# danielSanchezQ/dkg

Hardware: AMD Instinct MI355X
Metric: verified shares/sec (whole node) at n=1024,t=511; full-ceremony wall time (higher is better)
Workload: dtype u32 (GF(2^255-19), Z_l); 1 GPU; one DKG ceremony n=1024, t=511 (share gen + round-2/4 checks + finalise); n=1024, t=511, parallelism=single GPU, verify_streams=2, rounds_2_4_fused=True, degree_split=4, recombination=short lattice multipliers, recombination_addends=affine Niels, stepping_additions=dedicated (complete redo where exceptional)

## Files before the change

dkg_amd/csrc/kernels.hip:

```cpp
#ifdef DKG_FE_ILP
#define dkgk dkgk_ilp
#endif
#include "kernels.h"
#include "split.h"

#include <algorithm>
#include <cmath>
#include <type_traits>
#include "points.h"

namespace dkgk {

constexpr int COMB_WORDS = AFF_WORDS * COMB_ENTRIES;

#ifndef DKG_DECODE_WAVES
#define DKG_DECODE_WAVES 2
#endif
__global__ __launch_bounds__(256, DKG_DECODE_WAVES) void k_decode(const uint32_t* __restrict__ comp, size_t count,
                                                uint32_t* __restrict__ ext, size_t stride,
                                                uint8_t* __restrict__ ok, size_t pm_N, size_t pm_npad,
                                                uint32_t nseg, uint32_t seg, size_t pm_L, size_t pm_pstride) {
  size_t e = (size_t)blockIdx.x * blockDim.x + threadIdx.x;
  if (e >= count) return;
  uint32_t w[8];
// ... 421 lines not shown
  tab += (size_t)blockIdx.y * G::WORDS;
  ge_p3 b, m;
  pt_load(b, ext, stride, e0 + blockIdx.y);
  for (int i = 0; i < BITS * w; i++) ge_dbl<true>(b, b);
  mul_small_uniform(m, b, (uint32_t)d);
  fe zi, x, y, t, d2;
  fe_ld(d2, ge_const::D2);
  fe_invert(zi, m.Z);
  fe_mul(x, m.X, zi);
  fe_mul(y, m.Y, zi);
  uint32_t* out = tab + ((size_t)w * G::ENTRIES + (d - 1)) * COMBW_STRIDE;
  fe_add(t, y, x);
  fe_carry(t, t);
#pragma unroll
  for (int i = 0; i < 10; i++) out[i] = t.v[i];
  fe_sub(t, y, x);
  fe_carry(t, t);
#pragma unroll
  for (int i = 0; i < 10; i++) out[10 + i] = t.v[i];
  fe_mul(t, x, y);
  fe_mul(t, t, d2);
#pragma unroll
  for (int i = 0; i < 10; i++) out[20 + i] = t.v[i];
  out[30] = 0;
  out[31] = 0;
}

static_assert(COMBW_WORDS * 4 == (size_t)(256 / DKG_COMBW_BITS + 1) * (1u << (DKG_COMBW_BITS - 1)) * 32 * 4,
              "runtime.hip COMBW_BYTES must match points.h");
static_assert(CombGeo<COMBW_BITS>::WORDS == COMBW_WORDS, "one comb geometry");

int fixed_base_windows() { return COMBW_WINDOWS; }

template <int BITS>
void build_combw_r(const uint32_t* ext, size_t stride, size_t e0, uint32_t* tab, hipStream_t stream, size_t count) {
  if (!count) return;
  using G = CombGeo<BITS>;
  hipLaunchKernelGGL(k_build_combw<BITS>, dim3((unsigned)G::WINDOWS, (unsigned)count, G::ENTRIES / comb_build_bs<BITS>()),
                     dim3(comb_build_bs<BITS>()), 0, stream, ext, stride, e0, tab);
}

void build_combw(const uint32_t* ext, size_t stride, size_t e0, uint32_t* tab, hipStream_t stream, size_t count) {
  build_combw_r<COMBW_BITS>(ext, stride, e0, tab, stream, count);
}

size_t key_comb_words() { return CombGeo<DKG_KEY_COMB_BITS>::WORDS; }
int key_comb_windows() { return CombGeo<DKG_KEY_COMB_BITS>::WINDOWS; }

void build_key_combs(const uint32_t* ext, size_t stride, size_t e0, uint32_t* tab, hipStream_t stream,
                     size_t count) {
  build_combw_r<DKG_KEY_COMB_BITS>(ext, stride, e0, tab, stream, count);
}

__global__ __launch_bounds__(256) void k_copy_pos(size_t width, size_t npad, size_t N, const uint32_t* __restrict__ C,
                                                  size_t kpos, uint32_t* __restrict__ e, size_t pstride) {
  const size_t dl = (size_t)blockIdx.x * blockDim.x + threadIdx.x;
  if (dl >= width) return;
  const size_t d = blockIdx.y * pstride + dl;
  const size_t S = N * npad;
#pragma unroll 8
  for (int w = 0; w < PT_WORDS; w++) e[w * S + d] = C[w * S + kpos * npad + d];
}

#ifndef DKG_STEP_NT
#define DKG_STEP_NT 0
#endif
#ifndef DKG_AFF_NT
#define DKG_AFF_NT 0
#endif
#ifndef DKG_BINOM_WAVE_NT
#define DKG_BINOM_WAVE_NT 0
#endif
#ifndef DKG_COMB_NT
#define DKG_COMB_NT 0
#endif
template <bool NT>
DKG_DEV void binom_st(uint32_t* p, uint32_t v) {
  if constexpr (NT) __builtin_nontemporal_store(v, p);
  else *p = v;
}
template <bool NT>
DKG_DEV void binom_pt_store(uint32_t* __restrict__ base, size_t stride, size_t e, const ge_p3& p) {
  if constexpr (NT) pt_store_nt(base, stride, e, p);
  else pt_store(base, stride, e, p);
}


#ifndef DKG_BINOM_STEP_WAVES
#define DKG_BINOM_STEP_WAVES 4
#endif
template <bool DED, bool NT, bool IL = false>
__global__ __launch_bounds__(64, IL ? 2 : DKG_BINOM_STEP_WAVES) void k_binom_step(int r, int k, size_t npad, size_t N,
                                                    const uint32_t* __restrict__ C,
                                                    const uint32_t* __restrict__ ein, uint32_t* __restrict__ eout,
                                                    size_t pstride, unsigned gx, unsigned last_piece,
                                                    int last_off, uint32_t* __restrict__ flags, size_t col_base,
                                                    size_t dreal, unsigned gw, int fany) {
  __shared__ uint32_t qs[PT_WORDS * 64];
  uint32_t* q = qs + threadIdx.x;
  const unsigned piece = blockIdx.x / gx, grp = blockIdx.x - piece * gx;
  const size_t d = piece * pstride + (size_t)grp * blockDim.x + threadIdx.x;
  const size_t S = N * npad;
  const int m = r - (int)blockIdx.y;
  if (m == 0) {
#pragma unroll 8
    for (int w = 0; w < PT_WORDS; w++) binom_st<NT>(eout + w * S + d, C[w * S + (size_t)k * npad + d]);
    return;
  }
  const int re = r - (piece == last_piece ? last_off : 0);
  if (m > re) return;
  {
    ge_p3 cur;
    pt_load(cur, ein, S, (size_t)m * npad + d);
    uint32_t keep = (m == re) ? 0u : 0xffffffffu;
    asm volatile("" : "+v"(keep));
    uint32_t* cw = reinterpret_cast<uint32_t*>(&cur);
#pragma unroll
    for (int w = 0; w < PT_WORDS; w++) cw[w] = (cw[w] & keep) | ((w == 10 || w == 20) ? ~keep & 1u : 0u);
    ge_cached cc;
    if constexpr (DED) ge_to_cached_ded(cc, cur);
    else ge_to_cached(cc, cur);
    lds_put_cached(q, cc);
  }
  __builtin_amdgcn_sched_barrier(0);
  ge_p3 x;
  pt_load(x, ein, S, (size_t)(m - 1) * npad + d);
  if constexpr (DED) {
    bool bad = false;
    ge_add_ded_lds(x, x, q);
    bad |= fe_tight_zero(x.Z);
    mul_small_ded_lds<IL || DKG_BINOM_IL != 0>(x, (uint32_t)m, q, bad);
    const size_t gcol = col_base + (size_t)grp * blockDim.x + threadIdx.x;
    const bool real = (gcol / gw) * 64 + (gcol % gw) % 64 < dreal;
    if (__ballot(bad && real) != 0 && threadIdx.x == 0)
      flags[fany ? 0 : (size_t)piece * (pstride / 64) + (col_base / 64) + grp] = 1u;
  } else {
    ge_add_lds<IL>(x, x, q, false);
    mul_small_lds<IL>(x, (uint32_t)m, q);
  }
  binom_pt_store<NT>(eout, S, (size_t)m * npad + d, x);
}

__global__ __launch_bounds__(64, 4) void k_binom_pair(int r, int k, size_t npad, size_t N,
                                                    const uint32_t* __restrict__ C,
                                                    const uint32_t* __restrict__ ein, uint32_t* __restrict__ eout,
                                                    size_t pstride, unsigned gx, unsigned last_piece,
                                                    int last_off) {
  __shared__ uint32_t xb[20 * 64];
  __shared__ uint32_t qs[PT_WORDS * 32];
  const int lane = threadIdx.x;
  const unsigned piece = blockIdx.x / gx, grp = blockIdx.x - piece * gx;
  const size_t d = piece * pstride + (size_t)grp * 32 + (lane >> 1);
  const size_t S = N * npad;
  const int m = r - (int)blockIdx.y;
  if (m == 0) {
    if (lane & 1) return;
#pragma unroll 8
    for (int w = 0; w < PT_WORDS; w++) eout[w * S + d] = C[w * S + (size_t)k * npad + d];
    return;
  }
  const int re = r - (piece == last_piece ? last_off : 0);
  if (m > re) return;
  const pair_ctx c{xb, qs + (lane >> 1), lane & 1, lane};
  {
    ge_p3 cur;
    pt_load(cur, ein, S, (size_t)m * npad + d);
    uint32_t keep = (m == re) ? 0u : 0xffffffffu;
    asm volatile("" : "+v"(keep));
    uint32_t* cw = reinterpret_cast<uint32_t*>(&cur);
#pragma unroll
    for (int w = 0; w < PT_WORDS; w++) cw[w] = (cw[w] & keep) | ((w == 10 || w == 20) ? ~keep & 1u : 0u);
    pair_put_cached(c, cur);
  }
  ge_p3 x;
  pt_load(x, ein, S, (size_t)(m - 1) * npad + d);
  ge_add_pair(x, x, c, false);
  mul_small_pair(x, (uint32_t)m, c);
  if (lane & 1) return;
  pt_store(eout, S, (size_t)m * npad + d, x);
}

void binom_step_pair(size_t r, size_t width, size_t npad, size_t N, const uint32_t* C, const uint32_t* in,
                     uint32_t* out, hipStream_t stream, size_t pieces, size_t pstride, size_t last_len) {
  const int last_off = (last_len && last_len < N) ? (int)(N - last_len) : 0;
  hipLaunchKernelGGL(k_binom_pair, dim3((unsigned)(width / 32 * pieces), (unsigned)(r + 1)), dim3(64), 0, stream,
                     (int)r, (int)(N - 1 - r), npad, N, C, in, out, pstride, (unsigned)(width / 32),
                     (unsigned)(pieces - 1), last_off);
}

void binom_init(size_t width, size_t npad, size_t N, const uint32_t* C, uint32_t* e0, hipStream_t stream,
                size_t pieces, size_t pstride) {
  hipLaunchKernelGGL(k_copy_pos, dim3((unsigned)((width + 255) / 256), (unsigned)pieces), dim3(256), 0, stream, width,
                     npad, N, C, N - 1, e0, pstride);
}

void binom_step(size_t r, size_t width, size_t npad, size_t N, const uint32_t* C, const uint32_t* in, uint32_t* out,
                hipStream_t stream, size_t pieces, size_t pstride, size_t last_len, uint32_t* flags, size_t col_base,
                size_t dreal, unsigned gw, bool flag_any, bool nt, bool il) {
  const int last_off = (last_len && last_len < N) ? (int)(N - last_len) : 0;
  const dim3 grid((unsigned)(width / 64 * pieces), (unsigned)(r + 1));
  auto go = [&](auto kern, uint32_t* fl, int fany) {
    hipLaunchKernelGGL(kern, grid, dim3(64), 0, stream, (int)r, (int)(N - 1 - r), npad, N, C, in, out, pstride,
                       (unsigned)(width / 64), (unsigned)(pieces - 1), last_off, fl, col_base, dreal, gw ? gw : 64u,
                       fany);
  };
  if (il) {
    if (flags && nt) go(k_binom_step<true, true, true>, flags, flag_any ? 1 : 0);
    else if (flags) go(k_binom_step<true, false, true>, flags, flag_any ? 1 : 0);
    else if (nt) go(k_binom_step<false, true, true>, nullptr, 0);
    else go(k_binom_step<false, false, true>, nullptr, 0);
    return;
  }
  if (flags && nt) go(k_binom_step<true, true>, flags, flag_any ? 1 : 0);
  else if (flags) go(k_binom_step<true, false>, flags, flag_any ? 1 : 0);
  else if (nt) go(k_binom_step<false, true>, nullptr, 0);
  else go(k_binom_step<false, false>, nullptr, 0);
}

#ifndef DKG_BINOM_WAVE_CARRY
#define DKG_BINOM_WAVE_CARRY 1
#endif
#ifndef DKG_BINOM_WAVE_WAVES
#define DKG_BINOM_WAVE_WAVES 3
#endif
template <bool CARRY, bool PF, bool DED>
__global__ __launch_bounds__(64, PF ? 2 : (CARRY ? DKG_BINOM_WAVE_WAVES : 4)) void k_binom_wave(int L, size_t npad,
                                                                           const uint32_t* __restrict__ C,
                                                                           uint32_t* e, size_t pstride, unsigned gx,
                                                                           unsigned last_piece, int last_off,
                                                                           uint32_t* eT, uint32_t* __restrict__ flags,
                                                                           size_t col_base, size_t dreal, unsigned gw) {
  static_assert(!PF || CARRY, "the prefetch runs on the carried schedule");
  static_assert(!DED || (CARRY && !PF), "the dedicated pass runs on the carried schedule");
  __shared__ uint32_t qs[PT_WORDS * 64];
  uint32_t* q = qs + threadIdx.x;
  const unsigned piece = blockIdx.x / gx, grp = blockIdx.x - piece * gx;
  const size_t fidx = (size_t)piece * (pstride / 64) + (col_base / 64) + grp;
  if (!DED && flags && !flags[fidx]) return;
  const size_t col0 = piece * pstride + (size_t)grp * 64;
  uint32_t* eb = e + col0;
  const uint32_t* cb = C + col0;
  const uint32_t lane = threadIdx.x;
  const size_t S = (size_t)L * npad;
  const int off = piece == last_piece ? last_off : 0;
  bool bad = false;
  const size_t gcol = col_base + (size_t)grp * 64 + lane;
  const bool real = (gcol / gw) * 64 + (gcol % gw) % 64 < dreal;
  uint32_t* e_top = (L == 1 && eT) ? eT + col0 : eb;
#pragma unroll 8
  for (int w = 0; w < PT_WORDS; w++) e_top[w * S + lane] = cb[w * S + (size_t)(L - 1) * npad + lane];
#pragma unroll 1
  for (int r = 1; r < L; r++) {
    asm volatile("s_waitcnt vmcnt(0)" ::: "memory");
    const int re = r - off;
    ge_p3 carry, nx;
    if constexpr (CARRY) ge_identity(carry);
    if constexpr (PF) {
// ... 41 lines not shown
        if (DKG_BINOM_WAVE_NT) pt_store_nt(eo, S, (size_t)m * npad + lane, x);
        else pt_store(eo, S, (size_t)m * npad + lane, x);
      } else {
        uint32_t* eo = eT + col0 * L;
        asm volatile("" : "+s"(eo));
        pt_store(eo, S, (size_t)lane * L + m, x);
      }
    }
    if (r + 1 < L || !eT) {
#pragma unroll 8
      for (int w = 0; w < PT_WORDS; w++) eb[w * S + lane] = cb[w * S + (size_t)(L - 1 - r) * npad + lane];
    } else {
      uint32_t* eo = eT + col0 * L;
#pragma unroll 8
      for (int w = 0; w < PT_WORDS; w++) eo[w * S + (size_t)lane * L] = cb[w * S + lane];
    }
  }
  if constexpr (DED) {
    if (__ballot(bad && real) != 0 && lane == 0) flags[fidx] = 1u;
  }
}

uint32_t* binomial_wave(size_t width, size_t npad, size_t N, const uint32_t* C, uint32_t* e, hipStream_t stream,
                        size_t pieces, size_t pstride, size_t last_len, uint32_t* eT, bool prefetch,
                        uint32_t* flags, size_t col_base, size_t dreal, unsigned gw) {
  const int last_off = (last_len && last_len < N) ? (int)(N - last_len) : 0;
  const dim3 grid((unsigned)(width / 64 * pieces));
  const unsigned gx = (unsigned)(width / 64), lp = (unsigned)(pieces - 1);
  if (!gw) gw = 64;
  if (prefetch) {
    hipLaunchKernelGGL((k_binom_wave<true, true, false>), grid, dim3(64), 0, stream, (int)N, npad, C, e, pstride, gx,
                       lp, last_off, eT, nullptr, col_base, dreal, gw);
  } else if (flags && DKG_BINOM_WAVE_CARRY) {
    hipLaunchKernelGGL((k_binom_wave<true, false, true>), grid, dim3(64), 0, stream, (int)N, npad, C, e, pstride, gx,
                       lp, last_off, eT, flags, col_base, dreal, gw);
    hipLaunchKernelGGL((k_binom_wave<true, false, false>), grid, dim3(64), 0, stream, (int)N, npad, C, e, pstride,
                       gx, lp, last_off, eT, flags, col_base, dreal, gw);
  } else {
    hipLaunchKernelGGL((k_binom_wave<DKG_BINOM_WAVE_CARRY != 0, false, false>), grid, dim3(64), 0, stream, (int)N,
                       npad, C, e, pstride, gx, lp, last_off, eT, nullptr, col_base, dreal, gw);
  }
  return e;
}

void binomial_wave_redo(size_t width, size_t npad, size_t N, const uint32_t* C, uint32_t* e, hipStream_t stream,
                        size_t pieces, size_t pstride, size_t last_len, uint32_t* flags, size_t col_base,
                        size_t dreal, unsigned gw) {
  const int last_off = (last_len && last_len < N) ? (int)(N - last_len) : 0;
  hipLaunchKernelGGL((k_binom_wave<true, false, false>), dim3((unsigned)(width / 64 * pieces)), dim3(64), 0, stream,
                     (int)N, npad, C, e, pstride, (unsigned)(width / 64), (unsigned)(pieces - 1), last_off, nullptr,
                     flags, col_base, dreal, gw ? gw : 64u);
}

uint32_t* binomial(size_t width, size_t npad, size_t N, const uint32_t* C, uint32_t* e0, uint32_t* e1,
                   hipStream_t stream, size_t pieces, size_t pstride, size_t last_len) {
  binom_init(width, npad, N, C, e0, stream, pieces, pstride);
  uint32_t* in = e0;
  uint32_t* out = e1;
  for (size_t r = 1; r < N; r++) {
    binom_step(r, width, npad, N, C, in, out, stream, pieces, pstride, last_len);
    std::swap(in, out);
  }
  return in;
}


__global__ __launch_bounds__(256) void k_to_column_major(size_t width, size_t npad, size_t N,
                                                         const uint32_t* __restrict__ e, uint32_t* __restrict__ eT,
                                                         size_t pstride) {
  __shared__ uint32_t tile[64][65];
  const size_t w = blockIdx.z % PT_WORDS, base = (blockIdx.z / PT_WORDS) * pstride;
  const size_t c0 = (size_t)blockIdx.x * 64, p0 = (size_t)blockIdx.y * 64;
  const size_t S = N * npad;
  const int tx = threadIdx.x & 63, ty = threadIdx.x >> 6;
#pragma unroll
  for (int i = 0; i < 16; i++) {
    const size_t p = p0 + ty + 4 * i, c = c0 + tx;
    if (p < N && c < width) tile[ty + 4 * i][tx] = e[w * S + p * npad + base + c];
  }
  __syncthreads();
#pragma unroll
  for (int i = 0; i < 16; i++) {
    const size_t c = c0 + ty + 4 * i, p = p0 + tx;
    if (p < N && c < width) eT[w * S + (base + c) * N + p] = tile[tx][ty + 4 * i];
  }
}

void to_column_major(size_t width, size_t npad, size_t N, const uint32_t* e, uint32_t* eT, size_t pieces,
                     size_t pstride, hipStream_t stream) {
  if (!width || !N) return;
  hipLaunchKernelGGL(k_to_column_major,
                     dim3((unsigned)((width + 63) / 64), (unsigned)((N + 63) / 64), (unsigned)(pieces * PT_WORDS)),
                     dim3(256), 0, stream, width, npad, N, e, eT, pstride);
}

__global__ __launch_bounds__(64) void k_zero_tests(size_t count, const uint32_t* __restrict__ limbs,
                                                   uint8_t* __restrict__ out) {
  const size_t e = (size_t)blockIdx.x * 64 + threadIdx.x;
  const bool live = e < count;
  fe a;
#pragma unroll
  for (int i = 0; i < 10; i++) a.v[i] = live ? limbs[10 * e + i] : 1u;
  bool guard = false;
  fe_zero_guard(guard, a, live);
  if (live) {
    out[3 * e] = fe_maybe_zero(a) ? 1 : 0;
    out[3 * e + 1] = fe_tight_zero(a) ? 1 : 0;
    out[3 * e + 2] = guard ? 1 : 0;
  }
}
void zero_tests(size_t count, const uint32_t* limbs, uint8_t* out, hipStream_t stream) {
  if (!count) return;
  hipLaunchKernelGGL(k_zero_tests, dim3((unsigned)((count + 63) / 64)), dim3(64), 0, stream, count, limbs, out);
}

DKG_DEV void fe_ld_raw(fe& r, const uint32_t* __restrict__ p) {
#pragma unroll
  for (int i = 0; i < 10; i++) r.v[i] = p[i];
// ... 1827 lines not shown
```

dkg_amd/csrc/kernels_decl.inc:

```
namespace dkgk {

void decode_points(const uint32_t* comp, size_t count, uint32_t* ext, size_t stride, uint8_t* ok,
                   hipStream_t stream);
void place_position_major(const uint32_t* src, size_t sstride, size_t D, size_t N, size_t npad, uint32_t* out,
                          hipStream_t stream, int nseg = 1, int seg = 0, size_t L = 0, size_t pstride = 0);
void gather_points(const uint32_t* src, size_t sstride, size_t step, size_t k0, size_t count, uint32_t* dst,
                   size_t dstride, hipStream_t stream);
void decode_position_major(const uint32_t* comp, size_t D, size_t N, size_t npad, uint32_t* out, uint8_t* ok,
                           hipStream_t stream, int nseg = 1, int seg = 0, size_t L = 0, size_t pstride = 0);
void fill_identity(size_t S, uint32_t* out, hipStream_t stream);
void check_both(size_t ndealers, size_t nrecv, size_t dealer0, size_t dealer_base, size_t nmod, const uint32_t* s,
                const uint32_t* sp, const uint32_t* R, const uint32_t* tab_g, const uint32_t* tab_h,
                const uint8_t* dok, uint8_t* dec2, uint8_t* dec4, hipStream_t stream, const uint32_t* scale = nullptr,
                size_t j0 = 0, size_t jn = 0, uint32_t* acc = nullptr);
void encode_points(const uint32_t* ext, size_t stride, size_t count, uint32_t* comp, hipStream_t stream);
void build_comb(const uint32_t* ext, size_t stride, size_t e0, uint32_t* tab, hipStream_t stream, size_t count = 1);
void build_combw(const uint32_t* ext, size_t stride, size_t e0, uint32_t* tab, hipStream_t stream, size_t count = 1);

void commit_position_major(size_t D, size_t N, const uint32_t* a, const uint32_t* b, const uint32_t* tab_g,
                           const uint32_t* tab_h, uint32_t* out, size_t W, size_t L, size_t pstride, uint32_t* A0,
                           size_t A0stride, hipStream_t stream);
void commit(size_t count, const uint32_t* a, const uint32_t* b, const uint32_t* tab_g,
            const uint32_t* tab_h, uint32_t* A_ext, uint32_t* E_ext, hipStream_t stream, size_t stride = 0);
void share_eval(size_t D, size_t n, size_t N, const uint32_t* a, const uint32_t* b, uint32_t* s,
                uint32_t* sp, hipStream_t stream);
void poly_eval(size_t D, size_t N, const uint32_t* coeffs, size_t M, const uint32_t* xs, uint32_t* out,
               hipStream_t stream);

uint32_t* binomial(size_t width, size_t npad, size_t N, const uint32_t* C, uint32_t* e0, uint32_t* e1,
                   hipStream_t stream, size_t pieces = 1, size_t pstride = 0, size_t last_len = 0);
void binom_init(size_t width, size_t npad, size_t N, const uint32_t* C, uint32_t* e0, hipStream_t stream,
                size_t pieces = 1, size_t pstride = 0);
void binom_step(size_t r, size_t width, size_t npad, size_t N, const uint32_t* C, const uint32_t* in, uint32_t* out,
                hipStream_t stream, size_t pieces = 1, size_t pstride = 0, size_t last_len = 0,
                uint32_t* flags = nullptr, size_t col_base = 0, size_t dreal = 0, unsigned gw = 64,
                bool flag_any = false,
                bool nt = false,
                bool il = false);
void binomial_wave_redo(size_t width, size_t npad, size_t N, const uint32_t* C, uint32_t* e, hipStream_t stream,
                        size_t pieces, size_t pstride, size_t last_len, uint32_t* flags, size_t col_base,
                        size_t dreal, unsigned gw);
uint32_t* binomial_wave(size_t width, size_t npad, size_t N, const uint32_t* C, uint32_t* e, hipStream_t stream,
                        size_t pieces = 1, size_t pstride = 0, size_t last_len = 0, uint32_t* eT = nullptr,
                        bool prefetch = false, uint32_t* flags = nullptr, size_t col_base = 0, size_t dreal = 0,
                        unsigned gw = 64);
void binom_step_pair(size_t r, size_t width, size_t npad, size_t N, const uint32_t* C, const uint32_t* in,
                     uint32_t* out, hipStream_t stream, size_t pieces = 1, size_t pstride = 0, size_t last_len = 0);
void to_column_major(size_t width, size_t npad, size_t N, const uint32_t* e, uint32_t* eT, size_t pieces,
                     size_t pstride, hipStream_t stream);
struct StepShape {
  size_t nblk, P, per, bs, maxbs;
};
StepShape stepping_shape(size_t N);
double step_occupancy(size_t bs, size_t maxbs);
bool stepping_whole_columns(size_t L, size_t pieces, size_t last_len);
double stepping_cycles(size_t cols, size_t N, size_t pieces, size_t last_len, bool whole, size_t nrecv = 0);
double stepping_waves_per_simd(size_t cols, size_t N, size_t pieces, size_t last_len, bool whole);
size_t stepping_flag_words(size_t ndealers, size_t pieces);
void zero_tests(size_t count, const uint32_t* limbs, uint8_t* out, hipStream_t stream);
enum {
  FE_OP_MUL, FE_OP_SQ, FE_OP_MUL2, FE_OP_SQ2, FE_OP_MUL_SMALL, FE_OP_CARRY, FE_OP_ADD, FE_OP_SUB, FE_OP_NEG,
  FE_OP_DBL, FE_OP_INVERT, FE_OP_POW22523, FE_OP_TOBYTES, FE_OP_FROMBYTES, FE_OP_ABS, FE_OP_COUNT
};
bool fe_ops_shape(int op, size_t* win, size_t* wout);
void fe_ops(int op, size_t count, const uint32_t* in, uint32_t* out, hipStream_t stream);
enum {
  SC_OP_REDUCE9, SC_OP_REDUCE256, SC_OP_REDUCE512, SC_OP_ADD, SC_OP_SUB, SC_OP_NEG, SC_OP_MUL_SMALL_ADD,
  SC_OP_HORNER2, SC_OP_LAZY, SC_OP_MONT_MUL, SC_OP_MUL, SC_OP_MONT_INV, SC_OP_RADIX16, SC_OP_COUNT
};
bool sc_ops_shape(int op, size_t* win, size_t* wout);
uint32_t sc_ops_lazy_steps();
void sc_ops(int op, size_t count, const uint32_t* in, uint32_t* out, hipStream_t stream);
bool stepping(size_t ndealers, size_t npad, size_t N, const uint32_t* e, size_t nrecv, uint32_t* R,
              uint32_t* stream_a, uint32_t* stream_b, hipStream_t stream, size_t pieces = 1, size_t pstride = 0,
              size_t last_len = 0, bool whole = true, uint32_t* flags = nullptr, size_t col0 = 0,
              size_t dreal = (size_t)-1, unsigned gw = 64, uint32_t* Rz = nullptr, uint32_t* tail_a = nullptr,
              uint32_t* tail_b = nullptr, bool r_scaled = false);
int stepping_tail_phases(size_t N, size_t nrecv, size_t pieces);
size_t stepping_tail_words(size_t ndealers, size_t N);
void combine(size_t width, size_t pstride, size_t pieces, size_t nrecv, const int8_t* digits, const int16_t* top,
             uint32_t* R, hipStream_t stream);
void combine_short(size_t width, size_t pstride, size_t pieces, size_t nrecv, const uint32_t* digits,
                   const int16_t* top, uint32_t* R, hipStream_t stream);
void affine_pieces(size_t width, size_t pstride, size_t pieces, size_t nrecv, const uint32_t* R, uint32_t* A,
                   hipStream_t stream, const uint32_t* Rz = nullptr, size_t j0 = 0, size_t jn = 0,
                   bool scaled = false);
void combine_short_aff(size_t width, size_t pstride, size_t pieces, size_t nrecv, const uint32_t* digits,
                       const int16_t* top, const uint32_t* A, uint32_t* R, hipStream_t stream, size_t j0 = 0,
                       size_t jn = 0);
void affine_pairs(size_t width, size_t pstride, size_t pieces, size_t nrecv, const uint32_t* R, uint32_t* A,
                  hipStream_t stream, size_t j0 = 0, size_t jn = 0, bool scaled = false);
constexpr uint32_t JSF_EV_NONE = 0xffu;
constexpr size_t JSF_EV_WORDS = 384;
void combine_short_jsf(size_t width, size_t pstride, size_t pieces, size_t nrecv, const uint32_t* digits,
                       const int16_t* top, const uint32_t* ev, const uint32_t* A, uint32_t* R, hipStream_t stream,
                       size_t j0 = 0, size_t jn = 0);
void check(size_t ndealers, size_t nrecv, size_t dealer_base, size_t recv_base, size_t nmod, int round,
           const uint32_t* s, const uint32_t* sp, const uint32_t* R, const uint32_t* tab_g,
           const uint32_t* tab_h, const uint8_t* dealer_ok, uint8_t* decision, hipStream_t stream,
           const uint32_t* scale = nullptr);
// ... 144 lines not shown
```

dkg_amd/csrc/runtime.hip:

```cpp
#include <hip/hip_runtime.h>

#include <cstdio>
#include <cstdlib>
#include <cstring>
#include <algorithm>
#include <array>
#include <iterator>
#include <map>
#include <memory>
#include <optional>
#include <string>
#include <thread>
#include <unordered_map>
#include <unordered_set>
#include <vector>

#include "../../include/dkg_amd.h"
#include "host_crypto.h"
#include "kernels.h"
#include "kernels_ilp.h"
#include "comb_build.h"
#include "seat_finalise.h"
#include "seat_deal.h"

struct dkg_ctx {
  int device = 0;
  hipStream_t stream = nullptr;
  std::string err;
  std::map<std::string, std::pair<void*, size_t>> bufs;
  std::map<std::string, std::pair<void*, size_t>> hbufs;
  uint32_t* tab_g = nullptr;
  uint32_t* tab_h = nullptr;
  uint32_t* tab_gw = nullptr;
  uint32_t* tab_hw = nullptr;
  uint8_t h[32] = {0};
  bool have_h = false;
  size_t threshold = 0, nr_members = 0;
  hipEvent_t ev[8] = {};
  struct PhaseMark {
    const char* tag;
    int phase;
  };
  std::vector<hipEvent_t> phase_pool;
  std::vector<PhaseMark> phase_marks;
  int receiver_chunk = 0;
  int last_receiver_chunk = 0;
  size_t ps_slab = 0;
  std::map<std::array<size_t, 4>, dkg_receiver_plan> recv_plans;
  std::map<std::array<size_t, 3>, std::vector<uint32_t>> pair_digits;
  static constexpr int MAX_SUB = 8;
  int nsub = 2;
  hipStream_t sub[MAX_SUB] = {};
  hipEvent_t fork = nullptr, join[MAX_SUB] = {};
  hipStream_t side = nullptr;
  hipEvent_t side_fork = nullptr, shares_done = nullptr, pub_done = nullptr;
  hipEvent_t terms_done = nullptr;
  bool shares_pending = false;
  bool overlap = true;
  int split = 0;
  std::vector<uint8_t> key_tabs_pk;
  std::vector<uint8_t> key_tabs16_pk;
  int key_comb = 0;
  int last_key_comb = 0;
  int seat_deal = 0;
  int last_seat_deal = 0;
  int seat_eval = 0, seat_eval_chunk = 0;
  int last_seat_eval = 0, last_seat_eval_chunk = 0;
  uint8_t fb_base[32] = {0};
  bool fb_valid = false;
  int comb_build = 0;
  int last_comb_build = 0;
  hipEvent_t cb_ev[2] = {};
  int binom_mode = 0;
  int step_mode = 0;
  int check_mode = 0;
  int fe_mode = 0;
  int verify_mode = 0;
  size_t vinv_N = 0;
  size_t fallback_rows = 0;
  int last_split = 1;
  size_t last_split_len = 0;
  size_t ydig_n = 0, ydig_L = 0;
  int combine_mode = 0;
  int last_combine = 0;
  int last_binomial = 0;
  int step_formula = 0;
  uint32_t* last_step_flags = nullptr;
// ... 634 lines not shown
  auto checks = [&](size_t d0, size_t d1, hipStream_t st, size_t j0 = 0, size_t jn = 0) {
    if (d1 <= d0 || !segs[0].dec) return;
    wait_shares(ctx, st);
    if (defer_masks)
      for (int k = 0; k < nseg; k++)
        if (segs[k].extra_ok) dkgk::and_dealer_mask(d1 - d0, nseg, k, segs[k].extra_ok + d0, dok + d0 * nseg, st);
    const VerifySeg& g = segs[0];
    if (nseg == 2) {
      uint32_t* acc = ctx->check_mode == 1 ? buf<uint32_t>(ctx, "v.acc", PTB * D * n) + d0 * n * PT_WORDS_H : nullptr;
      dkgk::check_both(d1 - d0, n, d0, g.dealer_base, g.self_mod ? g.self_mod : n, g.s, g.sp, R,
                       ctx->tab_gw, ctx->tab_hw, dok, g.dec, segs[1].dec, st, sscale, j0, jn, acc);
    } else {
      dkgk::check(d1 - d0, n, g.dealer_base + d0, 0, g.self_mod ? g.self_mod : n, g.round, g.s + d0 * n * 8,
                  g.round == 2 ? g.sp + d0 * n * 8 : nullptr, R + d0 * n * PT_WORDS_H, ctx->tab_gw, ctx->tab_hw,
                  dok + d0, g.dec + d0 * n, st, sscale);
    }
  };
  const bool saturating = (W / 64) * (L / 2) >= 4 * 1024;
  const bool long_stepping = (double)W * (double)L * (double)n >= 5e7 && npad >= 512;
  const size_t nsub = (saturating || long_stepping) ? std::min<size_t>(ctx->nsub, groups) : 1;
  const bool per_wave = ctx->binom_mode == 4 || ctx->binom_mode == 5 ||
                        (ctx->binom_mode == 0 && L > 1 && (double)npad / 64 * U >= DKG_BINOM_WAVE_GROUPS);
  ctx->last_binomial = per_wave ? 1 : 0;
  uint32_t* bflags = nullptr;
  const bool wave_ded = per_wave && DKG_BINOM_WAVE_DED && ctx->binom_mode != 5 &&
                        !(ctx->binom_mode == 0 && DKG_BINOM_WAVE_PF);
  const bool step_ded = !per_wave && ((DKG_BINOM_STEP_DED == 1 && ctx->binom_step_ded && ctx->binom_any) ||
                                      DKG_BINOM_STEP_DED == 2);
  if (ctx->step_formula == 0 && (wave_ded || (step_ded && DKG_BINOM_STEP_DED == 2))) {
    bflags = buf<uint32_t>(ctx, "v.bflags", 4 * (W / 64));
    HCK(hipMemsetAsync(bflags, 0, 4 * (W / 64), home));
  }
  ctx->last_bflags = bflags;
  ctx->last_bflag_words = bflags ? W / 64 : 0;
  uint32_t* bany = step_ded && DKG_BINOM_STEP_DED == 1 && ctx->step_formula == 0 ? ctx->binom_any : nullptr;
  const bool tails = ctx->step_mode != 3 && dkgk::stepping_tail_phases(L, n, U) > 1;
  uint32_t* tail_a = tails ? buf<uint32_t>(ctx, "v.tail_a", 4 * dkgk::stepping_tail_words(npad, L)) : nullptr;
  uint32_t* tail_b = tails ? buf<uint32_t>(ctx, "v.tail_b", 4 * dkgk::stepping_tail_words(npad, L)) : nullptr;
  auto chunk = [&](size_t g0, size_t g1, hipStream_t st, bool tm) {
    const size_t c0 = g0 * gw, w = (g1 - g0) * gw;
    if (defer_r1) {
      const size_t d0 = g0 * 64, d1 = std::min(D, g1 * 64);
      dkgk::commit_position_major(d1 - d0, N, ctx->r1_a + d0 * N * 8, ctx->r1_b + d0 * N * 8, ctx->tab_gw,
                                  ctx->tab_hw, Cpm + c0, W, L, npad, ctx->r1_A0 + d0, D, st);
    }
    if (tm) phase_mark(ctx, st, tag, -1);
    const uint32_t* e;
    if (per_wave) {
      e = dkgk::binomial_wave(w, W, L, Cpm + c0, e0 + c0, st, U, npad, Lr,
                              DKG_BINOM_WAVE_COLMAJOR ? eT + c0 * L : nullptr,
                              ctx->binom_mode == 5 || (ctx->binom_mode == 0 && DKG_BINOM_WAVE_PF), bflags, c0, D,
                              (unsigned)gw);
    } else {
      dkgk::binom_init(w, W, L, Cpm + c0, e0 + c0, st, U, npad);
      uint32_t *bin = e0 + c0, *bout = e1 + c0;
      for (size_t r = 1; r < L; r++) {
        const double wps = (double)npad / 64 * U * (r + 1) / 1024;
        const bool ilp = use_ilp(ctx, wps < binom_ilp_waves());
        const bool pair = ctx->binom_mode == 2 || ((ctx->binom_mode == 0 || ctx->binom_mode == 3) &&
                                                   wps < DKG_BINOM_PAIR_WAVES);
        if (pair)
          (ilp ? dkgk_ilp::binom_step_pair : dkgk::binom_step_pair)(r, w, W, L, Cpm + c0, bin, bout, st, U, npad,
                                                                    Lr);
        else
          (ilp ? dkgk_ilp::binom_step : dkgk::binom_step)(r, w, W, L, Cpm + c0, bin, bout, st, U, npad, Lr,
                                                          bany ? bany : bflags, c0, D, (unsigned)gw, bany != nullptr,
                                                          binom_nt(r, npad * U), !ilp && wps < binom_il_waves());
        std::swap(bin, bout);
      }
      e = bin;
      if (bflags && DKG_BINOM_STEP_DED == 2)
        dkgk::binomial_wave_redo(w, W, L, Cpm + c0, bin, st, U, npad, Lr, bflags, c0, D, (unsigned)gw);
    }
    if (tm) phase_mark(ctx, st, tag, VP_BINOMIAL);
    if (!per_wave || !DKG_BINOM_WAVE_COLMAJOR)
      dkgk::to_column_major(w, W, L, e, eT + c0 * L, U, npad, st);
    uint32_t* fl = sflags ? sflags + dkgk::stepping_flag_words(c0, U) : nullptr;
    if (fl) HCK(hipMemsetAsync(fl, 0, 4 * dkgk::stepping_flag_words(w, U), st));
    auto step = step_ilp ? dkgk_ilp::stepping : dkgk::stepping;
    if (!step(w, W, L, eT + c0 * L, n, R + c0 * n * PT_WORDS_H, sa ? sa + c0 * n * 40 : nullptr,
              sb ? sb + c0 * n * 40 : nullptr, st, U, npad, Lr, whole, fl, c0, D, (unsigned)gw,
              Rz ? Rz + c0 * n * 10 : nullptr, tail_a, tail_b, r_scaled))
      throw Fail{DKG_E_ARG};
    if (tm) phase_mark(ctx, st, tag, VP_STEPPING);
    if (jsf) {
      dkgk::affine_pairs(w, npad, U, n, R + c0 * n * PT_WORDS_H, Aff + c0 * n * AFFP_WORDS_H, st, 0, 0, r_scaled);
      dkgk::combine_short_jsf(w, npad, U, n, sdig, stop, sev, Aff + c0 * n * AFFP_WORDS_H, R + c0 * n * PT_WORDS_H, st);
    } else if (short_mult && Aff) {
      dkgk::affine_pieces(w, npad, U, n, R + c0 * n * PT_WORDS_H, Aff + c0 * n * AFFP_WORDS_H, st, Rz + c0 * n * 10, 0,
                          0, r_scaled);
      dkgk::combine_short_aff(w, npad, U, n, sdig, stop, Aff + c0 * n * AFFP_WORDS_H, R + c0 * n * PT_WORDS_H, st);
    } else if (short_mult) dkgk::combine_short(w, npad, U, n, sdig, stop, R + c0 * n * PT_WORDS_H, st);
    else dkgk::combine(w, npad, U, n, ydig, ytop, R + c0 * n * PT_WORDS_H, st);
    if (tm) phase_mark(ctx, st, tag, VP_COMBINE);
    checks(g0 * 64, std::min(D, g1 * 64), st);
    if (tm) phase_mark(ctx, st, tag, VP_CHECK);
  };
  if (nsub <= 1) {
    chunk(0, groups, home, timed);
  } else {
    HCK(hipEventRecord(ctx->fork, home));
    size_t g0 = 0;
    for (size_t c = 0; c < nsub; c++) {
      const size_t g1 = groups * (c + 1) / nsub;
      HCK(hipStreamWaitEvent(ctx->sub[c], ctx->fork, 0));
      chunk(g0, g1, ctx->sub[c], false);
      HCK(hipEventRecord(ctx->join[c], ctx->sub[c]));
      HCK(hipStreamWaitEvent(home, ctx->join[c], 0));
      g0 = g1;
    }
  }
  check_launch(ctx);
}

void verify_one(dkg_ctx* ctx, size_t n, size_t t, int round, size_t D, size_t dealer_base, const uint32_t* Ccomp,
                const uint32_t* s, const uint32_t* sp, uint8_t* dec, bool timed, const uint8_t* extra_ok = nullptr) {
  VerifySeg g{round, D, dealer_base, Ccomp, s, sp, dec, extra_ok};
  verify_device(ctx, n, t, &g, 1, timed, round == 2 ? "r2" : "r4");
}

template <typename F>
void verify_rounds_group(dkg_ctx* ctx, size_t n, size_t t, size_t D, size_t dealer_base, const uint32_t* Ecomp,
                         const uint32_t* Acomp, const uint32_t* s, const uint32_t* sp, uint8_t* dec2, uint8_t* dec4,
// ... 1669 lines not shown
int dkg_ctx_clock_probe(dkg_ctx* ctx, unsigned iters, double* sclk_mhz, double* busy_ms) {
  return guarded(ctx, [&] {
    if (!sclk_mhz || !busy_ms || !iters) return DKG_E_ARG;
    int cus = 0, wall_khz = 0;
    HCK(hipDeviceGetAttribute(&cus, hipDeviceAttributeMultiprocessorCount, ctx->device));
    HCK(hipDeviceGetAttribute(&wall_khz, hipDeviceAttributeWallClockRate, ctx->device));
    if (cus <= 0 || wall_khz <= 0) return DKG_E_DEVICE;
    const size_t waves = (size_t)cus * 16;
    unsigned long long* d = buf<unsigned long long>(ctx, "clock_probe", 2 * 8 * waves);
    hipLaunchKernelGGL(k_clock_probe, dim3((unsigned)(waves / 4)), dim3(256), 0, ctx->stream, iters, d);
    check_launch(ctx);
    std::vector<unsigned long long> h(2 * waves);
    d2h(ctx, h.data(), d, 2 * 8 * waves);
    sync(ctx);
    std::vector<double> mhz(waves), ms(waves);
    for (size_t w = 0; w < waves; w++) {
      const double real_us = (double)h[2 * w + 1] / wall_khz * 1e3;
      mhz[w] = real_us > 0 ? (double)h[2 * w] / real_us : 0.0;
      ms[w] = real_us / 1e3;
    }
    std::nth_element(mhz.begin(), mhz.begin() + waves / 2, mhz.end());
    std::nth_element(ms.begin(), ms.begin() + waves / 2, ms.end());
    *sclk_mhz = mhz[waves / 2];
    *busy_ms = ms[waves / 2];
    return DKG_OK;
  });
}

int dkg_ctx_create(int device, dkg_ctx** out) {
  if (!out) return DKG_E_ARG;
  *out = nullptr;
  dkg_ctx* ctx = new dkg_ctx();
  ctx->device = device;
  int rc = guarded(ctx, [&] {
    int least = 0, greatest = 0;
    HCK(hipDeviceGetStreamPriorityRange(&least, &greatest));
    HCK(hipStreamCreateWithPriority(&ctx->stream, hipStreamNonBlocking, greatest));
    for (auto& e : ctx->ev) HCK(hipEventCreate(&e));
    ctx->phase_pool.resize(PHASE_POOL_MIN);
    for (auto& e : ctx->phase_pool) HCK(hipEventCreate(&e));
    for (auto& e : ctx->cb_ev) HCK(hipEventCreate(&e));
    for (auto& st : ctx->sub) HCK(hipStreamCreateWithPriority(&st, hipStreamNonBlocking, greatest));
    HCK(hipStreamCreateWithPriority(&ctx->side, hipStreamNonBlocking, least));
    HCK(hipEventCreateWithFlags(&ctx->side_fork, hipEventDisableTiming));
    HCK(hipEventCreateWithFlags(&ctx->shares_done, hipEventDisableTiming));
    HCK(hipEventCreateWithFlags(&ctx->pub_done, hipEventDisableTiming));
    HCK(hipEventCreateWithFlags(&ctx->terms_done, hipEventDisableTiming));
    HCK(hipEventCreateWithFlags(&ctx->fork, hipEventDisableTiming));
    for (auto& e : ctx->join) HCK(hipEventCreateWithFlags(&e, hipEventDisableTiming));
    HCK(hipMalloc(&ctx->tab_g, COMB_BYTES));
    HCK(hipMalloc(&ctx->tab_h, COMB_BYTES));
    HCK(hipMalloc(&ctx->tab_gw, COMBW_BYTES));
    HCK(hipMalloc(&ctx->tab_hw, COMBW_BYTES));
    bool ok = false;
    comb_for_point(ctx, BASEPOINT, ctx->tab_g, &ok, ctx->tab_gw);
    if (!ok) {
      ctx->err = "basepoint failed to decode on device";
      return DKG_E_DEVICE;
    }
    return DKG_OK;
  });
  if (rc != DKG_OK) {
    fprintf(stderr, "dkg_ctx_create: %s\n", ctx->err.c_str());
    dkg_ctx_destroy(ctx);
    return rc;
  }
  *out = ctx;
  return DKG_OK;
}

void dkg_ctx_destroy(dkg_ctx* ctx) {
  if (!ctx) return;
  (void)hipSetDevice(ctx->device);
  if (ctx->stream) (void)hipDeviceSynchronize();
  for (auto& kv : ctx->bufs) (void)hipFree(kv.second.first);
  for (auto& kv : ctx->hbufs) (void)hipHostFree(kv.second.first);
  if (ctx->tab_g) (void)hipFree(ctx->tab_g);
  if (ctx->tab_h) (void)hipFree(ctx->tab_h);
  if (ctx->tab_gw) (void)hipFree(ctx->tab_gw);
  if (ctx->tab_hw) (void)hipFree(ctx->tab_hw);
  for (auto& e : ctx->ev)
    if (e) (void)hipEventDestroy(e);
  for (auto& e : ctx->phase_pool)
    if (e) (void)hipEventDestroy(e);
  for (auto& e : ctx->cb_ev)
    if (e) (void)hipEventDestroy(e);
  for (auto& e : ctx->join)
    if (e) (void)hipEventDestroy(e);
  if (ctx->fork) (void)hipEventDestroy(ctx->fork);
  for (auto& st : ctx->sub)
    if (st) (void)hipStreamDestroy(st);
  if (ctx->stream) (void)hipStreamDestroy(ctx->stream);
  if (ctx->side) (void)hipStreamDestroy(ctx->side);
  if (ctx->side_fork) (void)hipEventDestroy(ctx->side_fork);
  if (ctx->shares_done) (void)hipEventDestroy(ctx->shares_done);
  if (ctx->pub_done) (void)hipEventDestroy(ctx->pub_done);
  if (ctx->terms_done) (void)hipEventDestroy(ctx->terms_done);
  delete ctx;
}

const char* dkg_ctx_last_error(const dkg_ctx* ctx) { return ctx ? ctx->err.c_str() : "null context"; }

double dkg_ctx_phase_ms(const dkg_ctx* ctx, const char* name) {
  if (!ctx || !name) return -1.0;
  auto it = ctx->phase_ms.find(name);
  return it == ctx->phase_ms.end() ? -1.0 : it->second;
// ... 3481 lines not shown
```

Before: 13.26 million verified shares/s.

## Drop binomial init copy; read identity and C row directly in step kernels

The separate k_copy_pos init kernel that copied a C row into the ping-pong buffer is removed. Step kernels now read the m==1 predecessor straight from C and load the top-row identity from a small preallocated identity buffer instead of masking loaded words. The grid drops the extra row except on the last step. This saves a launch and redundant global traffic per wave but changes buffer indexing, and the fe_zero_guard swap slightly alters the flagging logic.

```diff
diff --git a/dkg_amd/csrc/kernels.hip b/dkg_amd/csrc/kernels.hip
--- a/dkg_amd/csrc/kernels.hip
+++ b/dkg_amd/csrc/kernels.hip
@@ -497,16 +497,6 @@
   build_combw_r<DKG_KEY_COMB_BITS>(ext, stride, e0, tab, stream, count);
 }
 
-__global__ __launch_bounds__(256) void k_copy_pos(size_t width, size_t npad, size_t N, const uint32_t* __restrict__ C,
-                                                  size_t kpos, uint32_t* __restrict__ e, size_t pstride) {
-  const size_t dl = (size_t)blockIdx.x * blockDim.x + threadIdx.x;
-  if (dl >= width) return;
-  const size_t d = blockIdx.y * pstride + dl;
-  const size_t S = N * npad;
-#pragma unroll 8
-  for (int w = 0; w < PT_WORDS; w++) e[w * S + d] = C[w * S + kpos * npad + d];
-}
-
 #ifndef DKG_STEP_NT
 #define DKG_STEP_NT 0
 #endif
@@ -540,11 +530,13 @@
                                                     const uint32_t* __restrict__ ein, uint32_t* __restrict__ eout,
                                                     size_t pstride, unsigned gx, unsigned last_piece,
                                                     int last_off, uint32_t* __restrict__ flags, size_t col_base,
-                                                    size_t dreal, unsigned gw, int fany) {
+                                                    size_t dreal, unsigned gw, int fany,
+                                                    const uint32_t* __restrict__ ident) {
   __shared__ uint32_t qs[PT_WORDS * 64];
   uint32_t* q = qs + threadIdx.x;
   const unsigned piece = blockIdx.x / gx, grp = blockIdx.x - piece * gx;
-  const size_t d = piece * pstride + (size_t)grp * blockDim.x + threadIdx.x;
+  const size_t col0 = piece * pstride + (size_t)grp * blockDim.x;
+  const size_t d = col0 + threadIdx.x;
   const size_t S = N * npad;
   const int m = r - (int)blockIdx.y;
   if (m == 0) {
@@ -555,13 +547,12 @@
   const int re = r - (piece == last_piece ? last_off : 0);
   if (m > re) return;
   {
+    const bool top = m == re;
+    const uint32_t* cb = top ? ident : ein + (size_t)m * npad + col0;
+    size_t cs = top ? 64 : S;
+    asm volatile("" : "+s"(cb), "+s"(cs));
     ge_p3 cur;
-    pt_load(cur, ein, S, (size_t)m * npad + d);
-    uint32_t keep = (m == re) ? 0u : 0xffffffffu;
-    asm volatile("" : "+v"(keep));
-    uint32_t* cw = reinterpret_cast<uint32_t*>(&cur);
-#pragma unroll
-    for (int w = 0; w < PT_WORDS; w++) cw[w] = (cw[w] & keep) | ((w == 10 || w == 20) ? ~keep & 1u : 0u);
+    pt_load(cur, cb, cs, threadIdx.x);
     ge_cached cc;
     if constexpr (DED) ge_to_cached_ded(cc, cur);
     else ge_to_cached(cc, cur);
@@ -569,11 +560,15 @@
   }
   __builtin_amdgcn_sched_barrier(0);
   ge_p3 x;
-  pt_load(x, ein, S, (size_t)(m - 1) * npad + d);
+  {
+    const uint32_t* xb = (m == 1 ? C + (size_t)(k + 1) * npad : ein + (size_t)(m - 1) * npad) + col0;
+    asm volatile("" : "+s"(xb));
+    pt_load(x, xb, S, threadIdx.x);
+  }
   if constexpr (DED) {
     bool bad = false;
     ge_add_ded_lds(x, x, q);
-    bad |= fe_tight_zero(x.Z);
+    fe_zero_guard(bad, x.Z);
     mul_small_ded_lds<IL || DKG_BINOM_IL != 0>(x, (uint32_t)m, q, bad);
     const size_t gcol = col_base + (size_t)grp * blockDim.x + threadIdx.x;
     const bool real = (gcol / gw) * 64 + (gcol % gw) % 64 < dreal;
@@ -590,12 +585,13 @@
                                                     const uint32_t* __restrict__ C,
                                                     const uint32_t* __restrict__ ein, uint32_t* __restrict__ eout,
                                                     size_t pstride, unsigned gx, unsigned last_piece,
-                                                    int last_off) {
+                                                    int last_off, const uint32_t* __restrict__ ident) {
   __shared__ uint32_t xb[20 * 64];
   __shared__ uint32_t qs[PT_WORDS * 32];
   const int lane = threadIdx.x;
   const unsigned piece = blockIdx.x / gx, grp = blockIdx.x - piece * gx;
-  const size_t d = piece * pstride + (size_t)grp * 32 + (lane >> 1);
+  const size_t col0 = piece * pstride + (size_t)grp * 32;
+  const size_t d = col0 + (lane >> 1);
   const size_t S = N * npad;
   const int m = r - (int)blockIdx.y;
   if (m == 0) {
@@ -608,46 +604,46 @@
   if (m > re) return;
   const pair_ctx c{xb, qs + (lane >> 1), lane & 1, lane};
   {
+    const bool top = m == re;
+    const uint32_t* cb = top ? ident : ein + (size_t)m * npad + col0;
+    size_t cs = top ? 64 : S;
+    asm volatile("" : "+s"(cb), "+s"(cs));
     ge_p3 cur;
-    pt_load(cur, ein, S, (size_t)m * npad + d);
-    uint32_t keep = (m == re) ? 0u : 0xffffffffu;
-    asm volatile("" : "+v"(keep));
-    uint32_t* cw = reinterpret_cast<uint32_t*>(&cur);
-#pragma unroll
-    for (int w = 0; w < PT_WORDS; w++) cw[w] = (cw[w] & keep) | ((w == 10 || w == 20) ? ~keep & 1u : 0u);
+    pt_load(cur, cb, cs, (size_t)(lane >> 1));
     pair_put_cached(c, cur);
   }
   ge_p3 x;
-  pt_load(x, ein, S, (size_t)(m - 1) * npad + d);
+  {
+    const uint32_t* pb = (m == 1 ? C + (size_t)(k + 1) * npad : ein + (size_t)(m - 1) * npad) + col0;
+    asm volatile("" : "+s"(pb));
+    pt_load(x, pb, S, (size_t)(lane >> 1));
+  }
   ge_add_pair(x, x, c, false);
   mul_small_pair(x, (uint32_t)m, c);
   if (lane & 1) return;
   pt_store(eout, S, (size_t)m * npad + d, x);
 }
 
+static unsigned binom_rows(size_t r, size_t N) { return (unsigned)(r + 1 == N ? r + 1 : r); }
+
 void binom_step_pair(size_t r, size_t width, size_t npad, size_t N, const uint32_t* C, const uint32_t* in,
-                     uint32_t* out, hipStream_t stream, size_t pieces, size_t pstride, size_t last_len) {
+                     uint32_t* out, const uint32_t* ident, hipStream_t stream, size_t pieces, size_t pstride,
+                     size_t last_len) {
   const int last_off = (last_len && last_len < N) ? (int)(N - last_len) : 0;
-  hipLaunchKernelGGL(k_binom_pair, dim3((unsigned)(width / 32 * pieces), (unsigned)(r + 1)), dim3(64), 0, stream,
+  hipLaunchKernelGGL(k_binom_pair, dim3((unsigned)(width / 32 * pieces), binom_rows(r, N)), dim3(64), 0, stream,
                      (int)r, (int)(N - 1 - r), npad, N, C, in, out, pstride, (unsigned)(width / 32),
-                     (unsigned)(pieces - 1), last_off);
-}
-
-void binom_init(size_t width, size_t npad, size_t N, const uint32_t* C, uint32_t* e0, hipStream_t stream,
-                size_t pieces, size_t pstride) {
-  hipLaunchKernelGGL(k_copy_pos, dim3((unsigned)((width + 255) / 256), (unsigned)pieces), dim3(256), 0, stream, width,
-                     npad, N, C, N - 1, e0, pstride);
+                     (unsigned)(pieces - 1), last_off, ident);
 }
 
 void binom_step(size_t r, size_t width, size_t npad, size_t N, const uint32_t* C, const uint32_t* in, uint32_t* out,
-                hipStream_t stream, size_t pieces, size_t pstride, size_t last_len, uint32_t* flags, size_t col_base,
-                size_t dreal, unsigned gw, bool flag_any, bool nt, bool il) {
+                const uint32_t* ident, hipStream_t stream, size_t pieces, size_t pstride, size_t last_len,
+                uint32_t* flags, size_t col_base, size_t dreal, unsigned gw, bool flag_any, bool nt, bool il) {
   const int last_off = (last_len && last_len < N) ? (int)(N - last_len) : 0;
-  const dim3 grid((unsigned)(width / 64 * pieces), (unsigned)(r + 1));
+  const dim3 grid((unsigned)(width / 64 * pieces), binom_rows(r, N));
   auto go = [&](auto kern, uint32_t* fl, int fany) {
     hipLaunchKernelGGL(kern, grid, dim3(64), 0, stream, (int)r, (int)(N - 1 - r), npad, N, C, in, out, pstride,
                        (unsigned)(width / 64), (unsigned)(pieces - 1), last_off, fl, col_base, dreal, gw ? gw : 64u,
-                       fany);
+                       fany, ident);
   };
   if (il) {
     if (flags && nt) go(k_binom_step<true, true, true>, flags, flag_any ? 1 : 0);
@@ -795,18 +791,6 @@
                      flags, col_base, dreal, gw ? gw : 64u);
 }
 
-uint32_t* binomial(size_t width, size_t npad, size_t N, const uint32_t* C, uint32_t* e0, uint32_t* e1,
-                   hipStream_t stream, size_t pieces, size_t pstride, size_t last_len) {
-  binom_init(width, npad, N, C, e0, stream, pieces, pstride);
-  uint32_t* in = e0;
-  uint32_t* out = e1;
-  for (size_t r = 1; r < N; r++) {
-    binom_step(r, width, npad, N, C, in, out, stream, pieces, pstride, last_len);
-    std::swap(in, out);
-  }
-  return in;
-}
-
 
 __global__ __launch_bounds__(256) void k_to_column_major(size_t width, size_t npad, size_t N,
                                                          const uint32_t* __restrict__ e, uint32_t* __restrict__ eT,
diff --git a/dkg_amd/csrc/kernels_decl.inc b/dkg_amd/csrc/kernels_decl.inc
--- a/dkg_amd/csrc/kernels_decl.inc
+++ b/dkg_amd/csrc/kernels_decl.inc
@@ -27,13 +27,10 @@
 void poly_eval(size_t D, size_t N, const uint32_t* coeffs, size_t M, const uint32_t* xs, uint32_t* out,
                hipStream_t stream);
 
-uint32_t* binomial(size_t width, size_t npad, size_t N, const uint32_t* C, uint32_t* e0, uint32_t* e1,
-                   hipStream_t stream, size_t pieces = 1, size_t pstride = 0, size_t last_len = 0);
-void binom_init(size_t width, size_t npad, size_t N, const uint32_t* C, uint32_t* e0, hipStream_t stream,
-                size_t pieces = 1, size_t pstride = 0);
 void binom_step(size_t r, size_t width, size_t npad, size_t N, const uint32_t* C, const uint32_t* in, uint32_t* out,
-                hipStream_t stream, size_t pieces = 1, size_t pstride = 0, size_t last_len = 0,
-                uint32_t* flags = nullptr, size_t col_base = 0, size_t dreal = 0, unsigned gw = 64,
+                const uint32_t* ident, hipStream_t stream, size_t pieces = 1, size_t pstride = 0,
+                size_t last_len = 0, uint32_t* flags = nullptr, size_t col_base = 0, size_t dreal = 0,
+                unsigned gw = 64,
                 bool flag_any = false,
                 bool nt = false,
                 bool il = false);
@@ -45,7 +42,8 @@
                         bool prefetch = false, uint32_t* flags = nullptr, size_t col_base = 0, size_t dreal = 0,
                         unsigned gw = 64);
 void binom_step_pair(size_t r, size_t width, size_t npad, size_t N, const uint32_t* C, const uint32_t* in,
-                     uint32_t* out, hipStream_t stream, size_t pieces = 1, size_t pstride = 0, size_t last_len = 0);
+                     uint32_t* out, const uint32_t* ident, hipStream_t stream, size_t pieces = 1, size_t pstride = 0,
+                     size_t last_len = 0);
 void to_column_major(size_t width, size_t npad, size_t N, const uint32_t* e, uint32_t* eT, size_t pieces,
                      size_t pstride, hipStream_t stream);
 struct StepShape {
diff --git a/dkg_amd/csrc/runtime.hip b/dkg_amd/csrc/runtime.hip
--- a/dkg_amd/csrc/runtime.hip
+++ b/dkg_amd/csrc/runtime.hip
@@ -33,6 +33,7 @@
   uint32_t* tab_h = nullptr;
   uint32_t* tab_gw = nullptr;
   uint32_t* tab_hw = nullptr;
+  uint32_t* ident = nullptr;
   uint8_t h[32] = {0};
   bool have_h = false;
   size_t threshold = 0, nr_members = 0;
@@ -773,7 +774,6 @@
                               ctx->binom_mode == 5 || (ctx->binom_mode == 0 && DKG_BINOM_WAVE_PF), bflags, c0, D,
                               (unsigned)gw);
     } else {
-      dkgk::binom_init(w, W, L, Cpm + c0, e0 + c0, st, U, npad);
       uint32_t *bin = e0 + c0, *bout = e1 + c0;
       for (size_t r = 1; r < L; r++) {
         const double wps = (double)npad / 64 * U * (r + 1) / 1024;
@@ -781,15 +781,15 @@
         const bool pair = ctx->binom_mode == 2 || ((ctx->binom_mode == 0 || ctx->binom_mode == 3) &&
                                                    wps < DKG_BINOM_PAIR_WAVES);
         if (pair)
-          (ilp ? dkgk_ilp::binom_step_pair : dkgk::binom_step_pair)(r, w, W, L, Cpm + c0, bin, bout, st, U, npad,
-                                                                    Lr);
+          (ilp ? dkgk_ilp::binom_step_pair : dkgk::binom_step_pair)(r, w, W, L, Cpm + c0, bin, bout, ctx->ident, st,
+                                                                    U, npad, Lr);
         else
-          (ilp ? dkgk_ilp::binom_step : dkgk::binom_step)(r, w, W, L, Cpm + c0, bin, bout, st, U, npad, Lr,
+          (ilp ? dkgk_ilp::binom_step : dkgk::binom_step)(r, w, W, L, Cpm + c0, bin, bout, ctx->ident, st, U, npad, Lr,
                                                           bany ? bany : bflags, c0, D, (unsigned)gw, bany != nullptr,
                                                           binom_nt(r, npad * U), !ilp && wps < binom_il_waves());
         std::swap(bin, bout);
       }
-      e = bin;
+      e = L == 1 ? Cpm + c0 : bin;
       if (bflags && DKG_BINOM_STEP_DED == 2)
         dkgk::binomial_wave_redo(w, W, L, Cpm + c0, bin, st, U, npad, Lr, bflags, c0, D, (unsigned)gw);
     }
@@ -2565,6 +2565,8 @@
     HCK(hipMalloc(&ctx->tab_h, COMB_BYTES));
     HCK(hipMalloc(&ctx->tab_gw, COMBW_BYTES));
     HCK(hipMalloc(&ctx->tab_hw, COMBW_BYTES));
+    ctx->ident = buf<uint32_t>(ctx, "ident", PTB * 64);
+    dkgk::fill_identity(64, ctx->ident, ctx->stream);
     bool ok = false;
     comb_for_point(ctx, BASEPOINT, ctx->tab_g, &ok, ctx->tab_gw);
     if (!ok) {
```

Result: no change. 13.29 million verified shares/s (median of 2 runs) (+0.2%).
